# zju3dv/NeuralRecon-W

Hardware: NVIDIA H100
Metric: training rays/sec (higher is better)
Workload: dtype bf16 (3-product split forward, plain bf16 backward, fp32 accumulate)

## Files before the change

neuralrecon-w_b200/csrc/gemm_tc.cu:

```cuda
#include <stdlib.h>

#include <mutex>
#include <unordered_map>
#include <vector>
#include <algorithm>
#include <stdio.h>

#include "gemm.h"
#include "epilogue_fast.cuh"

namespace nrw {

static constexpr int BM = 128;
static constexpr int BK = 64;
static constexpr int RING_BYTES = 192 * 1024;
static constexpr int MAX_STAGES = 8;
static constexpr int N_CONSUMER_WARPS = 8;
static constexpr int N_THREADS = 32 * N_CONSUMER_WARPS + 128;
static constexpr int PRODUCER_REGS = 40, CONSUMER_REGS = 232;
static constexpr int EPI_LD = 36;
static constexpr int EPI_WG_BYTES = 64 * EPI_LD * 4;
static constexpr int CS_BYTES = 1024;
static constexpr int BAR_TURN = 4;
static_assert(PRODUCER_REGS * 128 + CONSUMER_REGS * 32 * N_CONSUMER_WARPS <= 65536, "register file");
static constexpr int BAR_BYTES = 256;
static constexpr int SMEM_BYTES = 1024 + RING_BYTES + BAR_BYTES + 2 * EPI_WG_BYTES + CS_BYTES;
static_assert(SMEM_BYTES <= 232448, "dynamic shared memory limit of sm_90");
static_assert(4 * 2048 <= EPI_WG_BYTES, "the 2 KB per-warp epilogue tiles live in the warpgroup's staging tile");

struct TcParams {
  CUtensorMap tmA[3];
  CUtensorMap tmB[3];
  int M, N, K;
  int n_planes;
  int k_slices;
  int m_tiles, n_tiles;
  Epi epi;
  unsigned long long* prof;
};
#define NRW_PROF_T0(cond) const long long _t0 = (cond) ? clock64() : 0
#define NRW_PROF_ADD(cond, slot) \
  if (cond) atomicAdd(&p.prof[blockIdx.x * 16 + (slot)], (unsigned long long)(clock64() - _t0))

__device__ __forceinline__ uint32_t smem_u32(const void* p) {
  return static_cast<uint32_t>(__cvta_generic_to_shared(p));
}
__device__ __forceinline__ void mbar_init(uint32_t bar, uint32_t count) {
  asm volatile("mbarrier.init.shared::cta.b64 [%0], %1;" ::"r"(bar), "r"(count));
}
__device__ __forceinline__ void mbar_wait(uint32_t bar, uint32_t parity) {
  asm volatile(
      "{\n"
      ".reg .pred p;\n"
      "WAIT_LOOP:\n"
      "mbarrier.try_wait.parity.shared::cta.b64 p, [%0], %1;\n"
      "@p bra.uni WAIT_DONE;\n"
      "bra.uni WAIT_LOOP;\n"
      "WAIT_DONE:\n"
      "}\n" ::"r"(bar),
      "r"(parity)
      : "memory");
}
__device__ __forceinline__ void mbar_arrive(uint32_t bar) {
  asm volatile("mbarrier.arrive.shared::cta.b64 _, [%0];" ::"r"(bar) : "memory");
}
__device__ __forceinline__ void mbar_arrive_expect_tx(uint32_t bar, uint32_t bytes) {
  asm volatile("mbarrier.arrive.expect_tx.shared::cta.b64 _, [%0], %1;" ::"r"(bar), "r"(bytes)
               : "memory");
}
__device__ __forceinline__ void tma_load_2d(uint32_t dst, const CUtensorMap* map, uint32_t bar,
                                            int x, int y) {
  asm volatile(
      "cp.async.bulk.tensor.2d.shared::cluster.global.mbarrier::complete_tx::bytes"
      " [%0], [%1, {%3, %4}], [%2];" ::"r"(dst),
      "l"(reinterpret_cast<uint64_t>(map)), "r"(bar), "r"(x), "r"(y)
      : "memory");
}
__device__ __forceinline__ void tma_prefetch_desc(const CUtensorMap* map) {
  asm volatile("prefetch.tensormap [%0];" ::"l"(reinterpret_cast<uint64_t>(map)) : "memory");
}
__device__ __forceinline__ void pdl_wait() { asm volatile("griddepcontrol.wait;" ::: "memory"); }
__device__ __forceinline__ void pdl_launch_dependents() { asm volatile("griddepcontrol.launch_dependents;" ::: "memory"); }
__device__ __forceinline__ void named_bar_sync(int id, int n) { asm volatile("bar.sync %0, %1;" ::"r"(id), "r"(n) : "memory"); }
__device__ __forceinline__ void named_bar_arrive(int id, int n) { asm volatile("bar.arrive %0, %1;" ::"r"(id), "r"(n) : "memory"); }
template <int R>
__device__ __forceinline__ void setmaxnreg_inc() { asm volatile("setmaxnreg.inc.sync.aligned.u32 %0;" ::"n"(R)); }
template <int R>
__device__ __forceinline__ void setmaxnreg_dec() { asm volatile("setmaxnreg.dec.sync.aligned.u32 %0;" ::"n"(R)); }
__device__ __forceinline__ void fence_proxy_async_smem() { asm volatile("fence.proxy.async.shared::cta;" ::: "memory"); }

__device__ __forceinline__ uint64_t make_gdesc(uint32_t saddr, uint32_t lbo_bytes, uint32_t sbo_bytes) {
  uint64_t d = 0;
  d |= (uint64_t)((saddr & 0x3FFFF) >> 4);
  d |= (uint64_t)((lbo_bytes >> 4) & 0x3FFF) << 16;
  d |= (uint64_t)((sbo_bytes >> 4) & 0x3FFF) << 32;
  d |= (uint64_t)1 << 62;
  return d;
}
__device__ __forceinline__ void wgmma_fence() { asm volatile("wgmma.fence.sync.aligned;" ::: "memory"); }
__device__ __forceinline__ void wgmma_commit() { asm volatile("wgmma.commit_group.sync.aligned;" ::: "memory"); }
template <int N>
__device__ __forceinline__ void wgmma_wait() { asm volatile("wgmma.wait_group.sync.aligned %0;" ::"n"(N) : "memory"); }
template <int N>
__device__ __forceinline__ void acc_fence(float (&d)[N]) {
#pragma unroll
  for (int i = 0; i < N; ++i) asm volatile("" : "+f"(d[i])::"memory");
}

template <int BN, int TA, int TB>
__device__ __forceinline__ void wgmma_bf16(float (&d)[BN / 2], uint64_t da, uint64_t db, uint32_t accumulate);

template <>
__device__ __forceinline__ void wgmma_bf16<64, 0, 0>(float (&d)[32], uint64_t da, uint64_t db, uint32_t accumulate) {
  asm volatile(
      "{\n.reg .pred p;\nsetp.ne.b32 p, %34, 0;\n"
      "wgmma.mma_async.sync.aligned.m64n64k16.f32.bf16.bf16 "
      "{%0, %1, %2, %3, %4, %5, %6, %7, %8, %9, %10, %11, %12, %13, %14, %15, %16, %17, %18, %19, %20, %21, %22, %23, %24, %25, "
      "%26, %27, %28, %29, %30, %31}, %32, %33, p, 1, 1, 0, 0;\n}\n"
      : "+f"(d[0]), "+f"(d[1]), "+f"(d[2]), "+f"(d[3]), "+f"(d[4]), "+f"(d[5]), "+f"(d[6]), "+f"(d[7]), "+f"(d[8]), "+f"(d[9]),
        "+f"(d[10]), "+f"(d[11]), "+f"(d[12]), "+f"(d[13]), "+f"(d[14]), "+f"(d[15]), "+f"(d[16]), "+f"(d[17]), "+f"(d[18]),
        "+f"(d[19]), "+f"(d[20]), "+f"(d[21]), "+f"(d[22]), "+f"(d[23]), "+f"(d[24]), "+f"(d[25]), "+f"(d[26]), "+f"(d[27]),
        "+f"(d[28]), "+f"(d[29]), "+f"(d[30]), "+f"(d[31])
      : "l"(da), "l"(db), "r"(accumulate));
}
template <>
__device__ __forceinline__ void wgmma_bf16<64, 1, 1>(float (&d)[32], uint64_t da, uint64_t db, uint32_t accumulate) {
  asm volatile(
      "{\n.reg .pred p;\nsetp.ne.b32 p, %34, 0;\n"
      "wgmma.mma_async.sync.aligned.m64n64k16.f32.bf16.bf16 "
      "{%0, %1, %2, %3, %4, %5, %6, %7, %8, %9, %10, %11, %12, %13, %14, %15, %16, %17, %18, %19, %20, %21, %22, %23, %24, %25, "
      "%26, %27, %28, %29, %30, %31}, %32, %33, p, 1, 1, 1, 1;\n}\n"
      : "+f"(d[0]), "+f"(d[1]), "+f"(d[2]), "+f"(d[3]), "+f"(d[4]), "+f"(d[5]), "+f"(d[6]), "+f"(d[7]), "+f"(d[8]), "+f"(d[9]),
        "+f"(d[10]), "+f"(d[11]), "+f"(d[12]), "+f"(d[13]), "+f"(d[14]), "+f"(d[15]), "+f"(d[16]), "+f"(d[17]), "+f"(d[18]),
        "+f"(d[19]), "+f"(d[20]), "+f"(d[21]), "+f"(d[22]), "+f"(d[23]), "+f"(d[24]), "+f"(d[25]), "+f"(d[26]), "+f"(d[27]),
        "+f"(d[28]), "+f"(d[29]), "+f"(d[30]), "+f"(d[31])
      : "l"(da), "l"(db), "r"(accumulate));
}
#define NRW_WGMMA_N128(TA, TB)                                                                                                          \
  template <>                                                                                                                           \
  __device__ __forceinline__ void wgmma_bf16<128, TA, TB>(float (&d)[64], uint64_t da, uint64_t db, uint32_t accumulate) {              \
    asm volatile(                                                                                                                       \
        "{\n.reg .pred p;\nsetp.ne.b32 p, %66, 0;\n"                                                                                    \
        "wgmma.mma_async.sync.aligned.m64n128k16.f32.bf16.bf16 "                                                                        \
        "{%0, %1, %2, %3, %4, %5, %6, %7, %8, %9, %10, %11, %12, %13, %14, %15, %16, %17, %18, %19, %20, %21, %22, %23, %24, %25, "    \
        "%26, %27, %28, %29, %30, %31, %32, %33, %34, %35, %36, %37, %38, %39, %40, %41, %42, %43, %44, %45, %46, %47, %48, %49, %50, " \
        "%51, %52, %53, %54, %55, %56, %57, %58, %59, %60, %61, %62, %63}, %64, %65, p, 1, 1, " #TA ", " #TB ";\n}\n"                   \
        : "+f"(d[0]), "+f"(d[1]), "+f"(d[2]), "+f"(d[3]), "+f"(d[4]), "+f"(d[5]), "+f"(d[6]), "+f"(d[7]), "+f"(d[8]), "+f"(d[9]),     \
          "+f"(d[10]), "+f"(d[11]), "+f"(d[12]), "+f"(d[13]), "+f"(d[14]), "+f"(d[15]), "+f"(d[16]), "+f"(d[17]), "+f"(d[18]),        \
          "+f"(d[19]), "+f"(d[20]), "+f"(d[21]), "+f"(d[22]), "+f"(d[23]), "+f"(d[24]), "+f"(d[25]), "+f"(d[26]), "+f"(d[27]),        \
          "+f"(d[28]), "+f"(d[29]), "+f"(d[30]), "+f"(d[31]), "+f"(d[32]), "+f"(d[33]), "+f"(d[34]), "+f"(d[35]), "+f"(d[36]),        \
          "+f"(d[37]), "+f"(d[38]), "+f"(d[39]), "+f"(d[40]), "+f"(d[41]), "+f"(d[42]), "+f"(d[43]), "+f"(d[44]), "+f"(d[45]),        \
          "+f"(d[46]), "+f"(d[47]), "+f"(d[48]), "+f"(d[49]), "+f"(d[50]), "+f"(d[51]), "+f"(d[52]), "+f"(d[53]), "+f"(d[54]),        \
          "+f"(d[55]), "+f"(d[56]), "+f"(d[57]), "+f"(d[58]), "+f"(d[59]), "+f"(d[60]), "+f"(d[61]), "+f"(d[62]), "+f"(d[63])         \
        : "l"(da), "l"(db), "r"(accumulate));                                                                                           \
  }
NRW_WGMMA_N128(0, 0)
NRW_WGMMA_N128(1, 1)
#undef NRW_WGMMA_N128


template <int BN, int MN_MAJOR, int EK>
__global__ void __launch_bounds__(N_THREADS, 1) gemm_tc_kernel(const __grid_constant__ TcParams p) {
  static_assert(BN == 64 || BN == 128, "wgmma tile width");
  constexpr int A_TILE = BM * BK * 2;
  constexpr int B_TILE = BN * BK * 2;
  constexpr int WG_A = 64 * BK * 2;
  extern __shared__ uint8_t smem_raw[];
  uint8_t* smem = smem_raw + ((1024u - (smem_u32(smem_raw) & 1023u)) & 1023u);
  const int P = p.n_planes;
  const int stage_bytes = P * (A_TILE + B_TILE);
  int stages = RING_BYTES / stage_bytes;
  if (stages > MAX_STAGES) stages = MAX_STAGES;
  uint64_t* bars = reinterpret_cast<uint64_t*>(smem + RING_BYTES);
  const uint32_t bar_full = smem_u32(bars), bar_empty = smem_u32(bars + MAX_STAGES);
  float* epi_buf = reinterpret_cast<float*>(smem + RING_BYTES + BAR_BYTES);
  float* cs_buf = reinterpret_cast<float*>(smem + RING_BYTES + BAR_BYTES + 2 * EPI_WG_BYTES);
  const int warp = threadIdx.x >> 5, lane = threadIdx.x & 31;
  const long long t_kernel0 = clock64();

  if (warp == N_CONSUMER_WARPS && lane == 0) {
    for (int i = 0; i < P; ++i) {
      tma_prefetch_desc(&p.tmA[i]);
      tma_prefetch_desc(&p.tmB[i]);
    }
    for (int i = 0; i < MAX_STAGES; ++i) {
      mbar_init(bar_full + 8 * i, 1);
      mbar_init(bar_empty + 8 * i, 4);
    }
    asm volatile("fence.mbarrier_init.release.cluster;" ::: "memory");
  }
  if (threadIdx.x < 256) cs_buf[threadIdx.x] = 0.0f;
  __syncthreads();
  pdl_wait();
  pdl_launch_dependents();

  const int kb_total = (p.K + BK - 1) / BK;
  const int kb_per = (kb_total + p.k_slices - 1) / p.k_slices;
  const int n_items = p.m_tiles * p.n_tiles * p.k_slices;
  const int n_prod = (P == 1) ? 1 : (P == 2 ? 3 : 6);

  if (warp >= N_CONSUMER_WARPS) {
    setmaxnreg_dec<PRODUCER_REGS>();
    if (warp == N_CONSUMER_WARPS && lane == 0) {
      int s = 0;
      uint32_t ph = 0;
      for (int item = blockIdx.x; item < n_items; item += gridDim.x) {
        const int ks = item % p.k_slices;
        const int t = item / p.k_slices;
        const int n0 = (t % p.n_tiles) * BN, m0 = (t / p.n_tiles) * BM;
        const int kb0 = ks * kb_per, kb1 = min(kb_total, kb0 + kb_per);
        for (int kb = kb0; kb < kb1; ++kb) {
          {
            NRW_PROF_T0(p.prof != nullptr);
            mbar_wait(bar_empty + 8 * s, ph ^ 1);
            NRW_PROF_ADD(p.prof != nullptr, 0);
          }
          mbar_arrive_expect_tx(bar_full + 8 * s, stage_bytes);
          const uint32_t sa = smem_u32(smem + s * stage_bytes);
          const uint32_t sb = sa + P * A_TILE;
          for (int pl = 0; pl < P; ++pl) {
            if (MN_MAJOR == 0) {
              tma_load_2d(sa + pl * A_TILE, &p.tmA[pl], bar_full + 8 * s, kb * BK, m0);
              tma_load_2d(sb + pl * B_TILE, &p.tmB[pl], bar_full + 8 * s, kb * BK, n0);
            } else {
#pragma unroll
              for (int sl = 0; sl < BM / 64; ++sl)
                tma_load_2d(sa + pl * A_TILE + sl * (64 * BK * 2), &p.tmA[pl], bar_full + 8 * s,
                            m0 + 64 * sl, kb * BK);
#pragma unroll
              for (int sl = 0; sl < BN / 64; ++sl)
                tma_load_2d(sb + pl * B_TILE + sl * (64 * BK * 2), &p.tmB[pl], bar_full + 8 * s,
                            n0 + 64 * sl, kb * BK);
            }
          }
          if (++s == stages) { s = 0; ph ^= 1; }
        }
      }
    }
  } else {
    setmaxnreg_inc<CONSUMER_REGS>();
    const int wg = warp >> 2, wi = warp & 3;
    const uint32_t smem0 = smem_u32(smem);
    constexpr uint32_t LBO = MN_MAJOR ? (64 * BK * 2) : 16;
    constexpr uint32_t SBO = 1024;
    constexpr uint32_t KSTEP = MN_MAJOR ? (16 * 128) : 32;
    const uint64_t desc_hi = make_gdesc(0, LBO, SBO);
    float* stage_tile = epi_buf + wg * (EPI_WG_BYTES / 4);
    float* stg = stage_tile + wi * 512;
    const bool use_cs = p.epi.colsum != nullptr && !p.epi.atomic;
    float* cs_wg = cs_buf + 128 * wg;
    const int ctid = threadIdx.x & 127;
    const bool prof = p.prof != nullptr && wi == 0 && lane == 0;
    const int po = 8 * wg;
    int cs_n0 = -1;
    int s = 0;
    uint32_t ph = 0;
    for (int j = 0; blockIdx.x + j * gridDim.x < n_items; ++j) {
      const int item = blockIdx.x + j * gridDim.x;
      const int ks = item % p.k_slices;
      const int t = item / p.k_slices;
      const int n0 = (t % p.n_tiles) * BN, m0 = (t / p.n_tiles) * BM;
      const int kb0 = ks * kb_per, kb1 = min(kb_total, kb0 + kb_per);
      if ((j & 1) != wg) {
        for (int kb = kb0; kb < kb1; ++kb)
          if (++s == stages) { s = 0; ph ^= 1; }
        continue;
      }
      if (use_cs && n0 != cs_n0) {
        if (cs_n0 >= 0) colsum_flush(cs_wg, p.epi.colsum, cs_n0, min(min(p.N, p.epi.n_store) - cs_n0, BN), ctid, 128, 2 + wg);
        cs_n0 = n0;
      }
      float acc[2][BN / 2];
#pragma unroll
      for (int h = 0; h < 2; ++h)
#pragma unroll
        for (int i = 0; i < BN / 2; ++i) acc[h][i] = 0.0f;
      if (j > 0) {
        NRW_PROF_T0(prof);
        named_bar_sync(BAR_TURN + wg, 256);
        NRW_PROF_ADD(prof, 3 + po);
      }
      int prev_s = -1;
      for (int kb = kb0; kb < kb1; ++kb) {
        {
          NRW_PROF_T0(prof);
          mbar_wait(bar_full + 8 * s, ph);
          NRW_PROF_ADD(prof, 1 + po);
        }
        const uint32_t sa = smem0 + s * stage_bytes;
        const uint32_t sb = smem0 + s * stage_bytes + P * A_TILE;
        wgmma_fence();
        for (int pr = 0; pr < n_prod; ++pr) {
          const int q = 4 * (n_prod - 1 - pr);
          const uint32_t pa = (0x021010u >> q) & 0xFu, pb = (0x201100u >> q) & 0xFu;
          const uint64_t da = desc_hi | (uint64_t)(((sa + pa * A_TILE) & 0x3FFFFu) >> 4);
          const uint64_t db = desc_hi | (uint64_t)(((sb + pb * B_TILE) & 0x3FFFFu) >> 4);
#pragma unroll
          for (int k = 0; k < BK / 16; ++k)
#pragma unroll
            for (int h = 0; h < 2; ++h)
              wgmma_bf16<BN, MN_MAJOR, MN_MAJOR>(acc[h], da + ((h * WG_A + k * KSTEP) >> 4), db + ((k * KSTEP) >> 4), 1u);
        }
        wgmma_commit();
        acc_fence(acc[0]);
        acc_fence(acc[1]);
        if (prev_s >= 0) {
          wgmma_wait<1>();
          acc_fence(acc[0]);
          acc_fence(acc[1]);
          if (lane == 0) mbar_arrive(bar_empty + 8 * prev_s);
        }
        prev_s = s;
        if (++s == stages) { s = 0; ph ^= 1; }
      }
      if (item + gridDim.x < n_items) named_bar_arrive(BAR_TURN + (wg ^ 1), 256);
      wgmma_wait<0>();
      acc_fence(acc[0]);
      acc_fence(acc[1]);
      if (prev_s >= 0 && lane == 0) mbar_arrive(bar_empty + 8 * prev_s);
      if (kb1 <= kb0) continue;
      NRW_PROF_T0(prof);
      if (prof) atomicAdd(&p.prof[blockIdx.x * 16 + 6 + po], 1ull);
      const int r0 = 16 * wi + (lane >> 2), c0 = 2 * (lane & 3);
      const int qq = wi & 1, cc = wi >> 1;
      const int n_cp = (min(BN, p.N - n0) + 31) / 32;
#pragma unroll
      for (int h = 0; h < 2; ++h) {
        const int m0w = m0 + 64 * h + 32 * qq;
        float hacc[4] = {0.0f, 0.0f, 0.0f, 0.0f};
#pragma unroll
        for (int cp = 0; cp < BN / 32; ++cp) {
          if (cp >= n_cp) break;
#pragma unroll
          for (int jj = 0; jj < 4; ++jj) {
            const int jf = 4 * cp + jj;
            *reinterpret_cast<float2*>(stage_tile + r0 * EPI_LD + 8 * jj + c0) = make_float2(acc[h][4 * jf], acc[h][4 * jf + 1]);
            *reinterpret_cast<float2*>(stage_tile + (r0 + 8) * EPI_LD + 8 * jj + c0) = make_float2(acc[h][4 * jf + 2], acc[h][4 * jf + 3]);
          }
          named_bar_sync(2 + wg, 128);
          float v[16];
          const float* src = stage_tile + (32 * qq + lane) * EPI_LD + 16 * cc;
#pragma unroll
          for (int i = 0; i < 4; ++i) {
            const float4 t4 = *reinterpret_cast<const float4*>(src + 4 * i);
            v[4 * i] = t4.x; v[4 * i + 1] = t4.y; v[4 * i + 2] = t4.z; v[4 * i + 3] = t4.w;
          }
          named_bar_sync(2 + wg, 128);
          const int nc = n0 + 32 * cp + 16 * cc;
          if (nc < p.N && m0w < p.M)
            epi_fast16<EK>(p.epi, stg, v, m0w, nc, p.M, p.N, lane, use_cs ? cs_wg + 32 * cp + 16 * cc : nullptr, hacc);
          named_bar_sync(2 + wg, 128);
        }
        if (EK == EK_FWD_HEAD && (lane & 3) == 0) {
          const int slot = (n0 / BN) * 2 + cc;
#pragma unroll
          for (int it = 0; it < 4; ++it) {
            const int row = m0w + it * 8 + (lane >> 2);
            if (row < p.M) p.epi.head_partial[(long long)row * 8 + slot] = hacc[it];
          }
        }
      }
      NRW_PROF_ADD(prof, 4 + po);
    }
    if (use_cs && cs_n0 >= 0) colsum_flush(cs_wg, p.epi.colsum, cs_n0, min(min(p.N, p.epi.n_store) - cs_n0, BN), ctid, 128, 2 + wg);
  }
  __syncthreads();
  if (p.prof && threadIdx.x == 0) atomicAdd(&p.prof[blockIdx.x * 16 + 5], (unsigned long long)(clock64() - t_kernel0));
}

typedef CUresult (*EncodeTiledFn)(CUtensorMap*, CUtensorMapDataType, cuuint32_t, void*, const cuuint64_t*,
                                  const cuuint64_t*, const cuuint32_t*, const cuuint32_t*,
                                  CUtensorMapInterleave, CUtensorMapSwizzle, CUtensorMapL2promotion,
                                  CUtensorMapFloatOOBfill);

static EncodeTiledFn get_encode() {
  static EncodeTiledFn fn = nullptr;
  static std::once_flag once;
  std::call_once(once, [] {
    void* sym = nullptr;
    cudaDriverEntryPointQueryResult qres;
    if (cudaGetDriverEntryPoint("cuTensorMapEncodeTiled", &sym, cudaEnableDefault, &qres) == cudaSuccess &&
        qres == cudaDriverEntryPointSuccess)
      fn = reinterpret_cast<EncodeTiledFn>(sym);
  });
  return fn;
}

struct MapKey {
  const void* ptr; long long inner, outer, ld; int box_inner, box_outer;
  bool operator==(const MapKey& o) const {
    return ptr == o.ptr && inner == o.inner && outer == o.outer && ld == o.ld &&
           box_inner == o.box_inner && box_outer == o.box_outer;
  }
};
struct MapKeyHash {
  size_t operator()(const MapKey& k) const {
    size_t h = std::hash<const void*>()(k.ptr);
    h = h * 1000003u ^ (size_t)k.inner; h = h * 1000003u ^ (size_t)k.outer;
    h = h * 1000003u ^ (size_t)k.ld; h = h * 1000003u ^ (size_t)(k.box_inner * 1024 + k.box_outer);
    return h;
  }
};
static std::unordered_map<MapKey, CUtensorMap, MapKeyHash> g_map_cache;
static std::mutex g_map_mutex;

static int make_map(CUtensorMap* out, const bf16* ptr, long long inner, long long outer, long long ld,
                    int box_inner, int box_outer, bool swizzle = true) {
  MapKey key{ptr, inner, outer, ld, swizzle ? box_inner : -box_inner, box_outer};
  {
    std::lock_guard<std::mutex> lk(g_map_mutex);
    auto it = g_map_cache.find(key);
    if (it != g_map_cache.end()) { *out = it->second; return NRW_OK; }
  }
  EncodeTiledFn enc = get_encode();
  NRW_CHECK(enc != nullptr, NRW_ERR_CUDA, "cuTensorMapEncodeTiled entry point unavailable");
  NRW_CHECK((reinterpret_cast<uintptr_t>(ptr) & 15) == 0 && (ld % 8) == 0, NRW_ERR_ARG,
            "TMA operand must be 16B aligned with ld %% 8 == 0 (ptr=%p ld=%lld)", (const void*)ptr, ld);
  cuuint64_t dims[2] = {(cuuint64_t)inner, (cuuint64_t)outer};
  cuuint64_t strides[1] = {(cuuint64_t)ld * 2};
  cuuint32_t box[2] = {(cuuint32_t)box_inner, (cuuint32_t)box_outer};
  cuuint32_t estr[2] = {1, 1};
  CUresult r = enc(out, CU_TENSOR_MAP_DATA_TYPE_BFLOAT16, 2, const_cast<bf16*>(ptr), dims, strides, box, estr,
                   CU_TENSOR_MAP_INTERLEAVE_NONE, swizzle ? CU_TENSOR_MAP_SWIZZLE_128B : CU_TENSOR_MAP_SWIZZLE_NONE,
                   CU_TENSOR_MAP_L2_PROMOTION_L2_256B, CU_TENSOR_MAP_FLOAT_OOB_FILL_NONE);
  NRW_CHECK(r == CUDA_SUCCESS, NRW_ERR_CUDA, "cuTensorMapEncodeTiled failed (%d) inner=%lld outer=%lld ld=%lld",
            (int)r, inner, outer, ld);
  std::lock_guard<std::mutex> lk(g_map_mutex);
  if (g_map_cache.size() > 65536) g_map_cache.clear();
  g_map_cache.emplace(key, *out);
  return NRW_OK;
}

static unsigned long long* g_prof_ptr = nullptr;
void gemm_tc_set_profile_buffer(unsigned long long* p) { g_prof_ptr = p; }
static long long g_tc_launches = 0;
long long gemm_tc_launch_count() { return g_tc_launches; }

static constexpr int MAX_DEV = 64;
static int current_device() {
  int dev = 0;
  cudaGetDevice(&dev);
  return (dev >= 0 && dev < MAX_DEV) ? dev : 0;
}

template <typename Kernel>
static cudaError_t launch_gemm(Kernel kernel, int grid, int block, cudaStream_t stream, const TcParams& p) {
  static const int pdl = getenv("NRW_PDL") ? atoi(getenv("NRW_PDL")) : 1;
  cudaLaunchConfig_t cfg;
  memset(&cfg, 0, sizeof(cfg));
  cfg.gridDim = dim3(grid, 1, 1);
  cfg.blockDim = dim3(block, 1, 1);
  cfg.dynamicSmemBytes = SMEM_BYTES;
  cfg.stream = stream;
  cudaLaunchAttribute attr[1];
  attr[0].id = cudaLaunchAttributeProgrammaticStreamSerialization;
  attr[0].val.programmaticStreamSerializationAllowed = 1;
  cfg.attrs = attr;
  cfg.numAttrs = pdl ? 1 : 0;
  return cudaLaunchKernelEx(&cfg, kernel, p);
}

template <int BN, int MN, int EK>
static int launch(const TcParams& p, int n_sm, int dev, cudaStream_t stream) {
  static bool attr_set[MAX_DEV] = {false};
  if (!attr_set[dev]) {
    NRW_CUDA_OK((cudaFuncSetAttribute(gemm_tc_kernel<BN, MN, EK>, cudaFuncAttributeMaxDynamicSharedMemorySize, SMEM_BYTES)));
    attr_set[dev] = true;
  }
  const int items = p.m_tiles * p.n_tiles * p.k_slices;
  const int grid = items < n_sm ? items : n_sm;
  NRW_CUDA_OK((launch_gemm(gemm_tc_kernel<BN, MN, EK>, grid, N_THREADS, stream, p)));
  NRW_LAUNCH_OK();
  ++g_tc_launches;
  return NRW_OK;
}

static int gemm_tc_impl(const GemmDesc& g, cudaStream_t stream);

struct TimedLaunch { cudaEvent_t e0, e1; double flops; double mma_flops; int M, N, K, P, mn, ks; unsigned epi; double bytes; };
static std::vector<TimedLaunch> g_timed;
static std::vector<cudaEvent_t> g_event_pool;
static bool g_timing_on = false;
void gemm_tc_timing_enable(bool on) { g_timing_on = on; }
static cudaEvent_t get_event() {
  if (!g_event_pool.empty()) { cudaEvent_t e = g_event_pool.back(); g_event_pool.pop_back(); return e; }
  cudaEvent_t e;
  cudaEventCreate(&e);
  return e;
}
int gemm_tc_timing_read(double* ms, double* flops, double* mma_flops, long long* launches, double* bytes) {
  double t = 0, f = 0, mf = 0, by = 0;
  FILE* dump = getenv("NRW_GEMM_TIMING_DUMP") ? fopen(getenv("NRW_GEMM_TIMING_DUMP"), "a") : nullptr;
  for (auto& L : g_timed) {
    NRW_CUDA_OK(cudaEventSynchronize(L.e1));
    float dt = 0;
    NRW_CUDA_OK(cudaEventElapsedTime(&dt, L.e0, L.e1));
    t += dt; f += L.flops; mf += L.mma_flops; by += L.bytes;
    g_event_pool.push_back(L.e0); g_event_pool.push_back(L.e1);
    if (dump) fprintf(dump, "%d,%d,%d,%d,%d,%d,%u,%.0f,%.4f\n", L.M, L.N, L.K, L.P, L.mn, L.ks, L.epi, L.bytes, dt);
  }
  if (dump) fclose(dump);
  *ms = t; *flops = f; *mma_flops = mf; *launches = (long long)g_timed.size();
  if (bytes) *bytes = by;
  g_timed.clear();
  return NRW_OK;
}

int gemm_tc(const GemmDesc& g, cudaStream_t stream) {
  if (!g_timing_on) return gemm_tc_impl(g, stream);
  TimedLaunch L;
  L.e0 = get_event(); L.e1 = get_event();
  L.flops = 2.0 * g.M * g.N * g.K;
  L.mma_flops = L.flops * n_products(g.n_planes);
  L.M = g.M; L.N = g.N; L.K = g.K; L.P = g.n_planes; L.mn = g.mn_major; L.ks = g.k_slices;
  const Epi& e = g.epi;
  const int q_bytes = e.aux_q_bcast ? 0 : e.aux_q.elem_bytes();
  L.epi = (e.out_pre ? 1u : 0u) | (e.out_f32 ? 2u : 0u) | (e.out2 ? 4u : 0u) | (e.n_planes ? 8u : 0u) | (e.aux_u.p ? 16u : 0u) |
          (q_bytes ? 32u : 0u) | (e.aux_add ? 64u : 0u) | (e.aux_relu ? 128u : 0u) | (e.atomic ? 256u : 0u) | (e.colsum ? 512u : 0u);
  const double mn = (double)g.M * (double)std::min(g.N, e.n_store);
  L.bytes = 2.0 * g.n_planes * ((double)g.M * g.K + (double)g.N * g.K) + (double)e.out_pre.elem_bytes() * g.M * g.N +
            mn * (4.0 * (e.out_f32 ? 1 : 0) + e.out2.elem_bytes() + q_bytes + e.aux_add.elem_bytes() + 2.0 * e.n_planes +
                  (e.aux_relu ? 2.0 : 0.0) + (e.aux_u.p ? 2.0 * e.aux_u_planes : 0.0));
  NRW_CUDA_OK(cudaEventRecord(L.e0, stream));
  const int rc = gemm_tc_impl(g, stream);
  NRW_CUDA_OK(cudaEventRecord(L.e1, stream));
  g_timed.push_back(L);
  return rc;
}
static int gemm_tc_impl(const GemmDesc& g, cudaStream_t stream) {
  NRW_CHECK(g.M > 0 && g.N > 0 && g.K > 0, NRW_ERR_ARG, "gemm_tc: empty problem %d %d %d", g.M, g.N, g.K);
  NRW_CHECK(g.n_planes >= 1 && g.n_planes <= 3, NRW_ERR_ARG, "gemm_tc: n_planes=%d", g.n_planes);
  NRW_CHECK(g.k_slices == 1 || g.epi.atomic, NRW_ERR_ARG, "gemm_tc: split-K needs an atomic epilogue");
  static int n_sm_dev[MAX_DEV] = {0};
  const int dev = current_device();
  if (!n_sm_dev[dev]) NRW_CUDA_OK(cudaDeviceGetAttribute(&n_sm_dev[dev], cudaDevAttrMultiProcessorCount, dev));
  const int n_sm = n_sm_dev[dev];
  const int BN = g.N <= 64 ? 64 : 128;
  TcParams p;
  memset(&p, 0, sizeof(p));
  p.M = g.M; p.N = g.N; p.K = g.K; p.n_planes = g.n_planes; p.k_slices = g.k_slices;
  p.m_tiles = cdiv(g.M, BM); p.n_tiles = cdiv(g.N, BN);
  p.epi = g.epi;
  p.prof = g_prof_ptr;
  for (int pl = 0; pl < g.n_planes; ++pl) {
    if (!g.mn_major) {
      NRW_CHECK(g.K % BK == 0, NRW_ERR_ARG, "gemm_tc: K=%d must be a multiple of %d (pad the operand)", g.K, BK);
      NRW_TRY(make_map(&p.tmA[pl], g.A.plane(pl), g.K, g.M, g.A.ld, BK, BM));
      NRW_TRY(make_map(&p.tmB[pl], g.B.plane(pl), g.K, g.N, g.B.ld, BK, BN));
    } else {
      NRW_TRY(make_map(&p.tmA[pl], g.A.plane(pl), g.M, g.K, g.A.ld, 64, BK));
      NRW_TRY(make_map(&p.tmB[pl], g.B.plane(pl), g.N, g.K, g.B.ld, 64, BK));
    }
  }
  const int ek = g.mn_major ? EK_GENERIC : pick_epi_kind(g.epi);
  NRW_CHECK(ek >= 0 && (ek != EK_FWD_HEAD || g.N == 512), NRW_ERR_ARG,
            "gemm_tc: the fused SDF-head epilogue needs N = 512, bias + softplus and no other output");
  if (g.mn_major) return BN == 64 ? launch<64, 1, EK_GENERIC>(p, n_sm, dev, stream) : launch<128, 1, EK_GENERIC>(p, n_sm, dev, stream);
  if (BN == 64) return launch<64, 0, EK_GENERIC>(p, n_sm, dev, stream);
  switch (ek) {
    case EK_FWD_SOFTPLUS: return launch<128, 0, EK_FWD_SOFTPLUS>(p, n_sm, dev, stream);
    case EK_FWD_RELU: return launch<128, 0, EK_FWD_RELU>(p, n_sm, dev, stream);
    case EK_FWD_NONE: return launch<128, 0, EK_FWD_NONE>(p, n_sm, dev, stream);
    case EK_FWD_HEAD: return launch<128, 0, EK_FWD_HEAD>(p, n_sm, dev, stream);
    case EK_GATE_FWD: return launch<128, 0, EK_GATE_FWD>(p, n_sm, dev, stream);
    case EK_TANGENT: return launch<128, 0, EK_TANGENT>(p, n_sm, dev, stream);
    case EK_REVERSE: return launch<128, 0, EK_REVERSE>(p, n_sm, dev, stream);
    case EK_RELU_BWD: return launch<128, 0, EK_RELU_BWD>(p, n_sm, dev, stream);
    default: return launch<128, 0, EK_GENERIC>(p, n_sm, dev, stream);
  }
}


static constexpr int FZ_ROWS = 64;
static constexpr int FZ_APLANE = FZ_ROWS * 512 * 2;
static constexpr int FZ_A = 2 * FZ_APLANE;
static constexpr int FZ_WG = 4;
static constexpr int FZ_WSTAGE = 64 * BK * 2;
static constexpr int FZ_NST = 3;
static constexpr int FZ_BAR = FZ_A + FZ_WG * FZ_NST * FZ_WSTAGE;
static constexpr int FZ_SMEM = 1024 + FZ_BAR + 256;
static constexpr int FZ_THREADS = 128 * FZ_WG;
static constexpr int FZ_POS_PER_TILE = 4 * (1 + 7 * 8);
static_assert(FZ_SMEM <= 232448, "dynamic shared memory limit of sm_90");

struct SdfFusedParams {
  CUtensorMap tmW[8][2];
  const float* bias[8];
  const float* head_w;
  const float* head_b;
  const float* pts;
  float* sdf;
  int M, n_tiles;
};

__device__ __forceinline__ float pe6_feature(const float (&x)[3], int f) {
  if (f < 3) return x[f];
  const int k = (f - 3) / 6, wi = (f - 3) % 6, c = wi % 3;
  float sn, cs;
  sincosf(x[c] * (float)(1 << k), &sn, &cs);
  return wi < 3 ? sn : cs;
}

__global__ void __launch_bounds__(FZ_THREADS, 1) sdf_fused_kernel(const __grid_constant__ SdfFusedParams p) {
  extern __shared__ uint8_t smem_raw[];
  uint8_t* smem = smem_raw + ((1024u - (smem_u32(smem_raw) & 1023u)) & 1023u);
  uint64_t* bars = reinterpret_cast<uint64_t*>(smem + FZ_BAR);
  const uint32_t w_full = smem_u32(bars);
  const int warp = threadIdx.x >> 5, lane = threadIdx.x & 31;
  const uint32_t smem0 = smem_u32(smem);
  const int g = warp >> 2, wi = warp & 3, et = threadIdx.x;
  const bool loader = wi == 0 && lane == 0;

  if (et == 0) {
    for (int l = 0; l < 8; ++l) { tma_prefetch_desc(&p.tmW[l][0]); tma_prefetch_desc(&p.tmW[l][1]); }
    for (int i = 0; i < FZ_WG * FZ_NST; ++i) mbar_init(w_full + 8 * i, 1);
    asm volatile("fence.mbarrier_init.release.cluster;" ::: "memory");
  }
  __syncthreads();
  pdl_wait();
  pdl_launch_dependents();

  auto load = [&](int pos) {
    const int tile = blockIdx.x + (pos / FZ_POS_PER_TILE) * gridDim.x;
    if (tile >= p.n_tiles) return;
    const int q = pos % FZ_POS_PER_TILE;
    const int l = q < 4 ? 0 : 1 + (q - 4) / 32, r = q < 4 ? q : (q - 4) % 32;
    const int kb = r >> 2, u = r & 3;
    const uint32_t st = g * FZ_NST + pos % FZ_NST;
    mbar_arrive_expect_tx(w_full + 8 * st, FZ_WSTAGE);
    tma_load_2d(smem0 + FZ_A + st * FZ_WSTAGE, &p.tmW[l][(u & 1) ? 0 : 1], w_full + 8 * st, kb * BK, 128 * g + 64 * (u >> 1));
  };
  if (loader)
    for (int i = 0; i < FZ_NST; ++i) load(i);

  {
    const int r0 = 16 * wi + (lane >> 2), c0 = 2 * (lane & 3);
    const uint64_t desc_hi = make_gdesc(0, 16, 1024);
    float* part = reinterpret_cast<float*>(smem);
    int pos = 0;
    for (int tile = blockIdx.x; tile < p.n_tiles; tile += gridDim.x) {
      const int m0 = tile * FZ_ROWS;
      *reinterpret_cast<uint4*>(smem + et * 16) = make_uint4(0, 0, 0, 0);
      *reinterpret_cast<uint4*>(smem + FZ_APLANE + et * 16) = make_uint4(0, 0, 0, 0);
      named_bar_sync(1, 128 * FZ_WG);
      if (et < 3 * FZ_ROWS) {
        const int r = et / 3, c = et % 3, m = m0 + r;
        const float x = m < p.M ? __ldg(p.pts + (long long)m * 3 + c) : 0.0f;
        auto put = [&](int j, float v) {
          const bf16 hi = __float2bfloat16_rn(v), lo = __float2bfloat16_rn(v - __bfloat162float(hi));
          const int off = r * 128 + (((j >> 3) ^ (r & 7)) << 4) + (j & 7) * 2;
          *reinterpret_cast<bf16*>(smem + off) = hi;
          *reinterpret_cast<bf16*>(smem + FZ_APLANE + off) = lo;
        };
        put(c, x);
#pragma unroll
        for (int k = 0; k < 6; ++k) {
          float sn, cs;
          sincosf(x * (float)(1 << k), &sn, &cs);
          put(3 + 6 * k + c, sn);
          put(3 + 6 * k + 3 + c, cs);
        }
      }
      fence_proxy_async_smem();
      named_bar_sync(1, 128 * FZ_WG);
      float hsum[2] = {0.0f, 0.0f};
      for (int l = 0; l < 8; ++l) {
        const int nkb = l == 0 ? 1 : 8;
        float acc0[32], acc1[32];
#pragma unroll
        for (int i = 0; i < 32; ++i) { acc0[i] = 0.0f; acc1[i] = 0.0f; }
        auto stage = [&](float (&ah)[32], const uint32_t sa, const int u) {
          const uint32_t st = g * FZ_NST + pos % FZ_NST;
          mbar_wait(w_full + 8 * st, (pos / FZ_NST) & 1);
          const uint64_t db = desc_hi | (uint64_t)(((smem0 + FZ_A + st * FZ_WSTAGE) & 0x3FFFFu) >> 4);
          wgmma_fence();
          if ((u & 1) == 0) {
            const uint64_t da = desc_hi | (uint64_t)((sa & 0x3FFFFu) >> 4);
#pragma unroll
            for (int k = 0; k < BK / 16; ++k) wgmma_bf16<64, 0, 0>(ah, da + 2 * k, db + 2 * k, 1u);
          } else {
#pragma unroll
            for (int pa = 1; pa >= 0; --pa) {
              const uint64_t da = desc_hi | (uint64_t)(((sa + pa * FZ_APLANE) & 0x3FFFFu) >> 4);
#pragma unroll
              for (int k = 0; k < BK / 16; ++k) wgmma_bf16<64, 0, 0>(ah, da + 2 * k, db + 2 * k, 1u);
            }
          }
          wgmma_commit();
          acc_fence(acc0);
          acc_fence(acc1);
          if (pos > 0) {
            wgmma_wait<1>();
            acc_fence(acc0);
            acc_fence(acc1);
            if (loader) load(pos + FZ_NST - 1);
          }
          ++pos;
        };
        for (int kb = 0; kb < nkb; ++kb) {
          const uint32_t sa = smem0 + kb * (FZ_ROWS * BK * 2);
          stage(acc0, sa, 0);
          stage(acc0, sa, 1);
          stage(acc1, sa, 2);
          stage(acc1, sa, 3);
        }
        wgmma_wait<0>();
        acc_fence(acc0);
        acc_fence(acc1);
        named_bar_sync(1, 128 * FZ_WG);
        const float* bias = p.bias[l];
        if (l == 7) {
#pragma unroll
          for (int j = 0; j < 16; ++j) {
            const int n = 128 * g + 8 * j + c0;
            const float2 b = __ldg(reinterpret_cast<const float2*>(bias + n));
            const float2 hw = __ldg(reinterpret_cast<const float2*>(p.head_w + n));
#pragma unroll
            for (int rr = 0; rr < 2; ++rr) {
              const float* a = j < 8 ? acc0 + 4 * j : acc1 + 4 * (j - 8);
              hsum[rr] = fmaf(softplus100(a[2 * rr] + b.x), hw.x, hsum[rr]);
              hsum[rr] = fmaf(softplus100(a[2 * rr + 1] + b.y), hw.y, hsum[rr]);
            }
          }
          break;
        }
        const float scale = l == 3 ? 0.70710678118654752440f : 1.0f;
        float x[2][3];
        if (l == 3 && g == 3) {
#pragma unroll
          for (int rr = 0; rr < 2; ++rr) {
            const int m = m0 + r0 + 8 * rr;
#pragma unroll
            for (int i = 0; i < 3; ++i) x[rr][i] = m < p.M ? __ldg(p.pts + (long long)m * 3 + i) : 0.0f;
          }
        }
#pragma unroll
        for (int j = 0; j < 16; ++j) {
          const int n = 128 * g + 8 * j + c0;
          const float2 b = __ldg(reinterpret_cast<const float2*>(bias + n));
#pragma unroll
          for (int rr = 0; rr < 2; ++rr) {
            const int row = r0 + 8 * rr;
            const float* a = j < 8 ? acc0 + 4 * j : acc1 + 4 * (j - 8);
            float w0 = softplus100(a[2 * rr] + b.x) * scale, w1 = softplus100(a[2 * rr + 1] + b.y) * scale;
            if (l == 3 && n + 1 >= 473) {
              if (n >= 473) w0 = pe6_feature(x[rr], n - 473) * 0.70710678118654752440f;
              w1 = pe6_feature(x[rr], n + 1 - 473) * 0.70710678118654752440f;
            }
            const __nv_bfloat162 hh = __floats2bfloat162_rn(w0, w1);
            const float2 hf = __bfloat1622float2(hh);
            const __nv_bfloat162 ll = __floats2bfloat162_rn(w0 - hf.x, w1 - hf.y);
            const int off = (n >> 6) * (FZ_ROWS * BK * 2) + row * 128 + ((((n & 63) >> 3) ^ (row & 7)) << 4) + (n & 7) * 2;
            *reinterpret_cast<__nv_bfloat162*>(smem + off) = hh;
            *reinterpret_cast<__nv_bfloat162*>(smem + FZ_APLANE + off) = ll;
          }
        }
        fence_proxy_async_smem();
        named_bar_sync(1, 128 * FZ_WG);
      }
#pragma unroll
      for (int rr = 0; rr < 2; ++rr) {
        hsum[rr] += __shfl_xor_sync(0xFFFFFFFFu, hsum[rr], 1);
        hsum[rr] += __shfl_xor_sync(0xFFFFFFFFu, hsum[rr], 2);
        if ((lane & 3) == 0) part[(r0 + 8 * rr) * 4 + g] = hsum[rr];
      }
      named_bar_sync(1, 128 * FZ_WG);
      if (et < FZ_ROWS) {
        const float4 a = *reinterpret_cast<const float4*>(part + et * 4);
        const int m = m0 + et;
        if (m < p.M) p.sdf[m] = ((a.x + a.y) + (a.z + a.w)) + __ldg(p.head_b);
      }
      named_bar_sync(1, 128 * FZ_WG);
    }
  }
}

int sdf_fused_forward(const SdfFusedDesc& d, cudaStream_t stream) {
  NRW_CHECK(d.M > 0 && d.pts && d.sdf && d.head_w && d.head_b, NRW_ERR_ARG, "sdf_fused_forward: bad arguments (M=%d)", d.M);
  SdfFusedParams p;
  memset(&p, 0, sizeof(p));
  for (int l = 0; l < 8; ++l) {
    const int K = l == 0 ? 64 : 512;
    NRW_CHECK(d.W[l].p && d.W[l].ld == K && d.bias[l], NRW_ERR_ARG, "sdf_fused_forward: layer %d needs packed [512 x %d] weights (ld=%d)", l, K, d.W[l].ld);
    for (int pl = 0; pl < 2; ++pl) NRW_TRY(make_map(&p.tmW[l][pl], d.W[l].plane(pl), K, 512, d.W[l].ld, BK, 64));
    p.bias[l] = d.bias[l];
  }
  p.head_w = d.head_w; p.head_b = d.head_b; p.pts = d.pts; p.sdf = d.sdf; p.M = d.M;
  p.n_tiles = cdiv(d.M, FZ_ROWS);
  static int n_sm_dev[MAX_DEV] = {0};
  static bool attr_set[MAX_DEV] = {false};
  const int dev = current_device();
  if (!n_sm_dev[dev]) NRW_CUDA_OK(cudaDeviceGetAttribute(&n_sm_dev[dev], cudaDevAttrMultiProcessorCount, dev));
  if (!attr_set[dev]) {
    NRW_CUDA_OK(cudaFuncSetAttribute(sdf_fused_kernel, cudaFuncAttributeMaxDynamicSharedMemorySize, FZ_SMEM));
    attr_set[dev] = true;
  }
  int grid = n_sm_dev[dev];
  if (p.n_tiles < grid) grid = p.n_tiles;
  static const int pdl = getenv("NRW_PDL") ? atoi(getenv("NRW_PDL")) : 1;
  cudaLaunchConfig_t cfg;
  memset(&cfg, 0, sizeof(cfg));
  cfg.gridDim = dim3(grid, 1, 1);
  cfg.blockDim = dim3(FZ_THREADS, 1, 1);
  cfg.dynamicSmemBytes = FZ_SMEM;
  cfg.stream = stream;
  cudaLaunchAttribute attr[1];
  attr[0].id = cudaLaunchAttributeProgrammaticStreamSerialization;
  attr[0].val.programmaticStreamSerializationAllowed = 1;
  cfg.attrs = attr;
  cfg.numAttrs = pdl ? 1 : 0;
  TimedLaunch L;
  if (g_timing_on) {
    L.e0 = get_event(); L.e1 = get_event();
    L.flops = 2.0 * d.M * 512.0 * (64.0 + 7.0 * 512.0);
    L.mma_flops = 3.0 * L.flops;
    L.M = d.M; L.N = 512; L.K = 64 + 7 * 512; L.P = 2; L.mn = 0; L.ks = 1; L.epi = 4096u;
    L.bytes = 16.0 * d.M;
    NRW_CUDA_OK(cudaEventRecord(L.e0, stream));
  }
  NRW_CUDA_OK(cudaLaunchKernelEx(&cfg, sdf_fused_kernel, p));
  if (g_timing_on) {
    NRW_CUDA_OK(cudaEventRecord(L.e1, stream));
    g_timed.push_back(L);
  }
  NRW_LAUNCH_OK();
  ++g_tc_launches;
  return NRW_OK;
}

}
```

Before: 34690.

## Add thread-block clusters with TMA multicast for MN-major GEMM operands

Launches the MN-major (backward weight-gradient) GEMMs as 2-CTA clusters along M. CTAs in a cluster that share an N tile split the B-operand load and multicast it, and each consumer releases ring stages on every peer's empty barrier. The goal is to cut global/L2 traffic for the shared operand. In exchange it adds cross-CTA barrier traffic and cluster synchronisation, may leave tail CTAs idle (guarded by a live check), and limits the grid to whatever cluster occupancy allows.

```diff
diff --git a/neuralrecon-w_b200/csrc/gemm_tc.cu b/neuralrecon-w_b200/csrc/gemm_tc.cu
--- a/neuralrecon-w_b200/csrc/gemm_tc.cu
+++ b/neuralrecon-w_b200/csrc/gemm_tc.cu
@@ -35,6 +35,7 @@
   int n_planes;
   int k_slices;
   int m_tiles, n_tiles;
+  int cm, cn;
   Epi epi;
   unsigned long long* prof;
 };
@@ -75,6 +76,28 @@
       " [%0], [%1, {%3, %4}], [%2];" ::"r"(dst),
       "l"(reinterpret_cast<uint64_t>(map)), "r"(bar), "r"(x), "r"(y)
       : "memory");
+}
+__device__ __forceinline__ void tma_load_2d_mc(uint32_t dst, const CUtensorMap* map, uint32_t bar, int x, int y, uint16_t mask) {
+  asm volatile(
+      "cp.async.bulk.tensor.2d.shared::cluster.global.mbarrier::complete_tx::bytes.multicast::cluster"
+      " [%0], [%1, {%3, %4}], [%2], %5;" ::"r"(dst),
+      "l"(reinterpret_cast<uint64_t>(map)), "r"(bar), "r"(x), "r"(y), "h"(mask)
+      : "memory");
+}
+__device__ __forceinline__ uint32_t cluster_rank() {
+  uint32_t r;
+  asm volatile("mov.u32 %0, %%cluster_ctarank;" : "=r"(r));
+  return r;
+}
+__device__ __forceinline__ void mbar_arrive_cluster(uint32_t bar, uint32_t rank) {
+  asm volatile(
+      "{\n.reg .b32 ra;\n"
+      "mapa.shared::cluster.u32 ra, %0, %1;\n"
+      "mbarrier.arrive.shared::cluster.b64 _, [ra];\n}\n" ::"r"(bar), "r"(rank)
+      : "memory");
+}
+__device__ __forceinline__ void cluster_sync() {
+  asm volatile("barrier.cluster.arrive.release.aligned;\nbarrier.cluster.wait.acquire.aligned;" ::: "memory");
 }
 __device__ __forceinline__ void tma_prefetch_desc(const CUtensorMap* map) {
   asm volatile("prefetch.tensormap [%0];" ::"l"(reinterpret_cast<uint64_t>(map)) : "memory");
@@ -177,6 +200,13 @@
   float* cs_buf = reinterpret_cast<float*>(smem + RING_BYTES + BAR_BYTES + 2 * EPI_WG_BYTES);
   const int warp = threadIdx.x >> 5, lane = threadIdx.x & 31;
   const long long t_kernel0 = clock64();
+  const int cm = MN_MAJOR ? p.cm : 1, cn = MN_MAJOR ? p.cn : 1, cs = cm * cn;
+  const uint32_t rank = cluster_rank();
+  const int rm = rank % cm, rn = rank / cm;
+  uint32_t mask_a = 0;
+  for (int j = 0; j < cn; ++j) mask_a |= 1u << (rm + cm * j);
+  const uint32_t mask_b = ((1u << cm) - 1u) << (cm * rn);
+  const uint32_t peers = mask_a | mask_b;
 
   if (warp == N_CONSUMER_WARPS && lane == 0) {
     for (int i = 0; i < P; ++i) {
@@ -185,52 +215,62 @@
     }
     for (int i = 0; i < MAX_STAGES; ++i) {
       mbar_init(bar_full + 8 * i, 1);
-      mbar_init(bar_empty + 8 * i, 4);
+      mbar_init(bar_empty + 8 * i, 4 * __popc(peers));
     }
     asm volatile("fence.mbarrier_init.release.cluster;" ::: "memory");
   }
   if (threadIdx.x < 256) cs_buf[threadIdx.x] = 0.0f;
-  __syncthreads();
+  if (cs > 1) cluster_sync();
+  else __syncthreads();
   pdl_wait();
   pdl_launch_dependents();
 
   const int kb_total = (p.K + BK - 1) / BK;
   const int kb_per = (kb_total + p.k_slices - 1) / p.k_slices;
-  const int n_items = p.m_tiles * p.n_tiles * p.k_slices;
+  const int n_tn = (p.n_tiles + cn - 1) / cn;
+  const int n_items = (p.m_tiles + cm - 1) / cm * n_tn * p.k_slices;
+  const int cid = blockIdx.x / cs, n_cl = gridDim.x / cs;
   const int n_prod = (P == 1) ? 1 : (P == 2 ? 3 : 6);
+  auto tile_of = [&](int item, int& m0, int& n0, int& kb0, int& kb1) {
+    const int ks = item % p.k_slices;
+    const int t = item / p.k_slices;
+    n0 = ((t % n_tn) * cn + rn) * BN;
+    m0 = ((t / n_tn) * cm + rm) * BM;
+    kb0 = ks * kb_per;
+    kb1 = min(kb_total, kb0 + kb_per);
+  };
 
   if (warp >= N_CONSUMER_WARPS) {
     setmaxnreg_dec<PRODUCER_REGS>();
     if (warp == N_CONSUMER_WARPS && lane == 0) {
+      const int a_pieces = MN_MAJOR ? 2 : cn, b_pieces = (MN_MAJOR && BN == 128) ? 2 : cm;
+      const int a_piece = A_TILE / a_pieces, b_piece = B_TILE / b_pieces;
       int s = 0;
       uint32_t ph = 0;
-      for (int item = blockIdx.x; item < n_items; item += gridDim.x) {
-        const int ks = item % p.k_slices;
-        const int t = item / p.k_slices;
-        const int n0 = (t % p.n_tiles) * BN, m0 = (t / p.n_tiles) * BM;
-        const int kb0 = ks * kb_per, kb1 = min(kb_total, kb0 + kb_per);
+      for (int item = cid; item < n_items; item += n_cl) {
+        int m0, n0, kb0, kb1;
+        tile_of(item, m0, n0, kb0, kb1);
         for (int kb = kb0; kb < kb1; ++kb) {
           {
             NRW_PROF_T0(p.prof != nullptr);
             mbar_wait(bar_empty + 8 * s, ph ^ 1);
             NRW_PROF_ADD(p.prof != nullptr, 0);
           }
-          mbar_arrive_expect_tx(bar_full + 8 * s, stage_bytes);
+          const uint32_t bar = bar_full + 8 * s;
+          mbar_arrive_expect_tx(bar, stage_bytes);
           const uint32_t sa = smem_u32(smem + s * stage_bytes);
           const uint32_t sb = sa + P * A_TILE;
           for (int pl = 0; pl < P; ++pl) {
-            if (MN_MAJOR == 0) {
-              tma_load_2d(sa + pl * A_TILE, &p.tmA[pl], bar_full + 8 * s, kb * BK, m0);
-              tma_load_2d(sb + pl * B_TILE, &p.tmB[pl], bar_full + 8 * s, kb * BK, n0);
-            } else {
-#pragma unroll
-              for (int sl = 0; sl < BM / 64; ++sl)
-                tma_load_2d(sa + pl * A_TILE + sl * (64 * BK * 2), &p.tmA[pl], bar_full + 8 * s,
-                            m0 + 64 * sl, kb * BK);
-#pragma unroll
-              for (int sl = 0; sl < BN / 64; ++sl)
-                tma_load_2d(sb + pl * B_TILE + sl * (64 * BK * 2), &p.tmB[pl], bar_full + 8 * s,
-                            n0 + 64 * sl, kb * BK);
+            for (int h = rn; h < a_pieces; h += cn) {
+              const int x = MN_MAJOR ? m0 + 64 * h : kb * BK, y = MN_MAJOR ? kb * BK : m0 + (BM / cn) * h;
+              if (cn == 1) tma_load_2d(sa + pl * A_TILE + h * a_piece, &p.tmA[pl], bar, x, y);
+              else tma_load_2d_mc(sa + pl * A_TILE + h * a_piece, &p.tmA[pl], bar, x, y, (uint16_t)mask_a);
+            }
+            for (int h = rm; h < b_pieces; h += cm) {
+              const int x = !MN_MAJOR ? kb * BK : (BN == 128 ? n0 + 64 * h : n0);
+              const int y = !MN_MAJOR ? n0 + (BN / cm) * h : (BN == 128 ? kb * BK : kb * BK + (BK / cm) * h);
+              if (cm == 1) tma_load_2d(sb + pl * B_TILE + h * b_piece, &p.tmB[pl], bar, x, y);
+              else tma_load_2d_mc(sb + pl * B_TILE + h * b_piece, &p.tmB[pl], bar, x, y, (uint16_t)mask_b);
             }
           }
           if (++s == stages) { s = 0; ph ^= 1; }
@@ -255,18 +295,22 @@
     int cs_n0 = -1;
     int s = 0;
     uint32_t ph = 0;
-    for (int j = 0; blockIdx.x + j * gridDim.x < n_items; ++j) {
-      const int item = blockIdx.x + j * gridDim.x;
-      const int ks = item % p.k_slices;
-      const int t = item / p.k_slices;
-      const int n0 = (t % p.n_tiles) * BN, m0 = (t / p.n_tiles) * BM;
-      const int kb0 = ks * kb_per, kb1 = min(kb_total, kb0 + kb_per);
+    auto release = [&](int st) {
+      if (cs == 1) mbar_arrive(bar_empty + 8 * st);
+      else
+        for (uint32_t m = peers; m; m &= m - 1) mbar_arrive_cluster(bar_empty + 8 * st, __ffs(m) - 1);
+    };
+    for (int j = 0; cid + j * n_cl < n_items; ++j) {
+      const int item = cid + j * n_cl;
+      int m0, n0, kb0, kb1;
+      tile_of(item, m0, n0, kb0, kb1);
       if ((j & 1) != wg) {
         for (int kb = kb0; kb < kb1; ++kb)
           if (++s == stages) { s = 0; ph ^= 1; }
         continue;
       }
-      if (use_cs && n0 != cs_n0) {
+      const bool live = m0 < p.M && n0 < p.N;
+      if (use_cs && live && n0 != cs_n0) {
         if (cs_n0 >= 0) colsum_flush(cs_wg, p.epi.colsum, cs_n0, min(min(p.N, p.epi.n_store) - cs_n0, BN), ctid, 128, 2 + wg);
         cs_n0 = n0;
       }
@@ -308,17 +352,17 @@
           wgmma_wait<1>();
           acc_fence(acc[0]);
           acc_fence(acc[1]);
-          if (lane == 0) mbar_arrive(bar_empty + 8 * prev_s);
+          if (lane == 0) release(prev_s);
         }
         prev_s = s;
         if (++s == stages) { s = 0; ph ^= 1; }
       }
-      if (item + gridDim.x < n_items) named_bar_arrive(BAR_TURN + (wg ^ 1), 256);
+      if (item + n_cl < n_items) named_bar_arrive(BAR_TURN + (wg ^ 1), 256);
       wgmma_wait<0>();
       acc_fence(acc[0]);
       acc_fence(acc[1]);
-      if (prev_s >= 0 && lane == 0) mbar_arrive(bar_empty + 8 * prev_s);
-      if (kb1 <= kb0) continue;
+      if (prev_s >= 0 && lane == 0) release(prev_s);
+      if (kb1 <= kb0 || !live) continue;
       NRW_PROF_T0(prof);
       if (prof) atomicAdd(&p.prof[blockIdx.x * 16 + 6 + po], 1ull);
       const int r0 = 16 * wi + (lane >> 2), c0 = 2 * (lane & 3);
@@ -364,7 +408,8 @@
     }
     if (use_cs && cs_n0 >= 0) colsum_flush(cs_wg, p.epi.colsum, cs_n0, min(min(p.N, p.epi.n_store) - cs_n0, BN), ctid, 128, 2 + wg);
   }
-  __syncthreads();
+  if (cs > 1) cluster_sync();
+  else __syncthreads();
   if (p.prof && threadIdx.x == 0) atomicAdd(&p.prof[blockIdx.x * 16 + 5], (unsigned long long)(clock64() - t_kernel0));
 }
 
@@ -443,33 +488,50 @@
   return (dev >= 0 && dev < MAX_DEV) ? dev : 0;
 }
 
-template <typename Kernel>
-static cudaError_t launch_gemm(Kernel kernel, int grid, int block, cudaStream_t stream, const TcParams& p) {
+static void launch_config(cudaLaunchConfig_t& cfg, cudaLaunchAttribute (&attr)[2], int grid, int cluster, cudaStream_t stream) {
   static const int pdl = getenv("NRW_PDL") ? atoi(getenv("NRW_PDL")) : 1;
-  cudaLaunchConfig_t cfg;
   memset(&cfg, 0, sizeof(cfg));
   cfg.gridDim = dim3(grid, 1, 1);
-  cfg.blockDim = dim3(block, 1, 1);
+  cfg.blockDim = dim3(N_THREADS, 1, 1);
   cfg.dynamicSmemBytes = SMEM_BYTES;
   cfg.stream = stream;
-  cudaLaunchAttribute attr[1];
-  attr[0].id = cudaLaunchAttributeProgrammaticStreamSerialization;
-  attr[0].val.programmaticStreamSerializationAllowed = 1;
+  int n = 0;
+  if (cluster > 1) {
+    attr[n].id = cudaLaunchAttributeClusterDimension;
+    attr[n].val.clusterDim.x = cluster;
+    attr[n].val.clusterDim.y = 1;
+    attr[n].val.clusterDim.z = 1;
+    ++n;
+  }
+  if (pdl) {
+    attr[n].id = cudaLaunchAttributeProgrammaticStreamSerialization;
+    attr[n].val.programmaticStreamSerializationAllowed = 1;
+    ++n;
+  }
   cfg.attrs = attr;
-  cfg.numAttrs = pdl ? 1 : 0;
-  return cudaLaunchKernelEx(&cfg, kernel, p);
+  cfg.numAttrs = n;
 }
 
 template <int BN, int MN, int EK>
 static int launch(const TcParams& p, int n_sm, int dev, cudaStream_t stream) {
   static bool attr_set[MAX_DEV] = {false};
+  static int max_clusters[MAX_DEV][5] = {};
+  auto kernel = gemm_tc_kernel<BN, MN, EK>;
   if (!attr_set[dev]) {
-    NRW_CUDA_OK((cudaFuncSetAttribute(gemm_tc_kernel<BN, MN, EK>, cudaFuncAttributeMaxDynamicSharedMemorySize, SMEM_BYTES)));
+    NRW_CUDA_OK((cudaFuncSetAttribute(kernel, cudaFuncAttributeMaxDynamicSharedMemorySize, SMEM_BYTES)));
     attr_set[dev] = true;
   }
-  const int items = p.m_tiles * p.n_tiles * p.k_slices;
-  const int grid = items < n_sm ? items : n_sm;
-  NRW_CUDA_OK((launch_gemm(gemm_tc_kernel<BN, MN, EK>, grid, N_THREADS, stream, p)));
+  const int cs = p.cm * p.cn;
+  cudaLaunchConfig_t cfg;
+  cudaLaunchAttribute attr[2];
+  if (cs > 1 && !max_clusters[dev][cs]) {
+    launch_config(cfg, attr, cs, cs, stream);
+    NRW_CUDA_OK((cudaOccupancyMaxActiveClusters(&max_clusters[dev][cs], kernel, &cfg)));
+    NRW_CHECK(max_clusters[dev][cs] > 0, NRW_ERR_CUDA, "gemm_tc: no cluster of %d CTAs fits the device", cs);
+  }
+  const int items = cdiv(p.m_tiles, p.cm) * cdiv(p.n_tiles, p.cn) * p.k_slices;
+  launch_config(cfg, attr, std::min(items, cs > 1 ? max_clusters[dev][cs] : n_sm) * cs, cs, stream);
+  NRW_CUDA_OK((cudaLaunchKernelEx(&cfg, kernel, p)));
   NRW_LAUNCH_OK();
   ++g_tc_launches;
   return NRW_OK;
@@ -477,7 +539,12 @@
 
 static int gemm_tc_impl(const GemmDesc& g, cudaStream_t stream);
 
-struct TimedLaunch { cudaEvent_t e0, e1; double flops; double mma_flops; int M, N, K, P, mn, ks; unsigned epi; double bytes; };
+static void gemm_cluster_shape(int m_tiles, bool mn_major, int* cm, int* cn) {
+  *cm = mn_major && m_tiles >= 2 ? 2 : 1;
+  *cn = 1;
+}
+
+struct TimedLaunch { cudaEvent_t e0, e1; double flops; double mma_flops; int M, N, K, P, mn, ks, cm, cn; unsigned epi; double bytes; };
 static std::vector<TimedLaunch> g_timed;
 static std::vector<cudaEvent_t> g_event_pool;
 static bool g_timing_on = false;
@@ -497,7 +564,7 @@
     NRW_CUDA_OK(cudaEventElapsedTime(&dt, L.e0, L.e1));
     t += dt; f += L.flops; mf += L.mma_flops; by += L.bytes;
     g_event_pool.push_back(L.e0); g_event_pool.push_back(L.e1);
-    if (dump) fprintf(dump, "%d,%d,%d,%d,%d,%d,%u,%.0f,%.4f\n", L.M, L.N, L.K, L.P, L.mn, L.ks, L.epi, L.bytes, dt);
+    if (dump) fprintf(dump, "%d,%d,%d,%d,%d,%d,%u,%.0f,%.4f,%d,%d\n", L.M, L.N, L.K, L.P, L.mn, L.ks, L.epi, L.bytes, dt, L.cm, L.cn);
   }
   if (dump) fclose(dump);
   *ms = t; *flops = f; *mma_flops = mf; *launches = (long long)g_timed.size();
@@ -513,6 +580,7 @@
   L.flops = 2.0 * g.M * g.N * g.K;
   L.mma_flops = L.flops * n_products(g.n_planes);
   L.M = g.M; L.N = g.N; L.K = g.K; L.P = g.n_planes; L.mn = g.mn_major; L.ks = g.k_slices;
+  gemm_cluster_shape(cdiv(g.M, BM), g.mn_major, &L.cm, &L.cn);
   const Epi& e = g.epi;
   const int q_bytes = e.aux_q_bcast ? 0 : e.aux_q.elem_bytes();
   L.epi = (e.out_pre ? 1u : 0u) | (e.out_f32 ? 2u : 0u) | (e.out2 ? 4u : 0u) | (e.n_planes ? 8u : 0u) | (e.aux_u.p ? 16u : 0u) |
@@ -540,16 +608,17 @@
   memset(&p, 0, sizeof(p));
   p.M = g.M; p.N = g.N; p.K = g.K; p.n_planes = g.n_planes; p.k_slices = g.k_slices;
   p.m_tiles = cdiv(g.M, BM); p.n_tiles = cdiv(g.N, BN);
+  gemm_cluster_shape(p.m_tiles, g.mn_major, &p.cm, &p.cn);
   p.epi = g.epi;
   p.prof = g_prof_ptr;
   for (int pl = 0; pl < g.n_planes; ++pl) {
     if (!g.mn_major) {
       NRW_CHECK(g.K % BK == 0, NRW_ERR_ARG, "gemm_tc: K=%d must be a multiple of %d (pad the operand)", g.K, BK);
-      NRW_TRY(make_map(&p.tmA[pl], g.A.plane(pl), g.K, g.M, g.A.ld, BK, BM));
-      NRW_TRY(make_map(&p.tmB[pl], g.B.plane(pl), g.K, g.N, g.B.ld, BK, BN));
+      NRW_TRY(make_map(&p.tmA[pl], g.A.plane(pl), g.K, g.M, g.A.ld, BK, BM / p.cn));
+      NRW_TRY(make_map(&p.tmB[pl], g.B.plane(pl), g.K, g.N, g.B.ld, BK, BN / p.cm));
     } else {
       NRW_TRY(make_map(&p.tmA[pl], g.A.plane(pl), g.M, g.K, g.A.ld, 64, BK));
-      NRW_TRY(make_map(&p.tmB[pl], g.B.plane(pl), g.N, g.K, g.B.ld, 64, BK));
+      NRW_TRY(make_map(&p.tmB[pl], g.B.plane(pl), g.N, g.K, g.B.ld, 64, BN == 128 ? BK : BK / p.cm));
     }
   }
   const int ek = g.mn_major ? EK_GENERIC : pick_epi_kind(g.epi);
@@ -814,7 +883,7 @@
     L.e0 = get_event(); L.e1 = get_event();
     L.flops = 2.0 * d.M * 512.0 * (64.0 + 7.0 * 512.0);
     L.mma_flops = 3.0 * L.flops;
-    L.M = d.M; L.N = 512; L.K = 64 + 7 * 512; L.P = 2; L.mn = 0; L.ks = 1; L.epi = 4096u;
+    L.M = d.M; L.N = 512; L.K = 64 + 7 * 512; L.P = 2; L.mn = 0; L.ks = 1; L.cm = 1; L.cn = 1; L.epi = 4096u;
     L.bytes = 16.0 * d.M;
     NRW_CUDA_OK(cudaEventRecord(L.e0, stream));
   }
```

Measured after the change: 35690 (median of 6 runs). +2.9%, better.
